# NVlabs/neuralrgbd

Measured on NVIDIA H100. Metric: depth frames/sec at 640x480x64-plane x4-view, higher is better.
Workload: dtype f32 (split-fp16 pair products: 22-bit significands, fp32 accumulate)

## Files before the change

neuralrgbd_b200/csrc/conv_f16.cu:

```cuda
#include <cuda.h>
#include <cuda_fp16.h>

#include "common.cuh"
#include "conv_wgmma.cuh"
#include "wgmma.cuh"
#include "../../include/nrgbd_dev.h"

namespace {

constexpr int WG_THREADS = 288;
constexpr int BKC = 32;

struct WgParams {
  float* y; const float* bias; double* stats;
  __half *y_hi, *y_lo;
  const float *aff_scale, *aff_shift, *res;
  const __half *res_hi, *res_lo;
  int relu;
  int N, Dz, Hy, Wx, tiles_x, tiles_y, n_tiles, wide;
  int cin_chunks, n_kz, n_tap, halo, in_stride, org_y, org_x;
  int Cout, c_first;
  int Dout, Hout, Wout, Cs_out, c_off, out_stride, out_off_y, out_off_x, leaky;
  int stages_a, stages_b, box_w, box_h;
  uint32_t a_tile_bytes, a_stage_bytes, a_tx_bytes, b_stage_bytes, wg_row16;
  uint32_t a_desc_hi, b_desc_hi;
  signed char dz[3];
  signed char dy[WG_MAX_TAP2D], dx[WG_MAX_TAP2D];
  unsigned short a_off16[WG_MAX_TAP2D];
  unsigned char wsel[3 * WG_MAX_TAP2D];
};

__device__ __forceinline__ uint32_t smem_u32(const void* p) { return (uint32_t)__cvta_generic_to_shared(p); }

__device__ __forceinline__ void mbar_init(uint32_t bar, uint32_t count) {
  asm volatile("mbarrier.init.shared::cta.b64 [%0], %1;" ::"r"(bar), "r"(count));
}
__device__ __forceinline__ void mbar_expect_tx(uint32_t bar, uint32_t bytes) {
  asm volatile("mbarrier.arrive.expect_tx.shared::cta.b64 _, [%0], %1;" ::"r"(bar), "r"(bytes) : "memory");
}
__device__ __forceinline__ void mbar_arrive(uint32_t bar) {
  asm volatile("mbarrier.arrive.shared::cta.b64 _, [%0];" ::"r"(bar) : "memory");
}
__device__ __forceinline__ void mbar_wait(uint32_t bar, uint32_t parity) {
  uint32_t done = 0;
#pragma unroll 1
  for (uint32_t it = 0; it < (1u << 27); ++it) {
    asm volatile(
        "{\n\t.reg .pred p;\n\t"
        "mbarrier.try_wait.parity.shared::cta.b64 p, [%1], %2;\n\t"
        "selp.b32 %0, 1, 0, p;\n\t}"
        : "=r"(done) : "r"(bar), "r"(parity) : "memory");
    if (done) return;
  }
  __trap();
}
__device__ __forceinline__ void tma_load_5d(uint32_t dst, const CUtensorMap* tm, uint32_t bar, int c0, int c1, int c2, int c3, int c4) {
  asm volatile(
      "cp.async.bulk.tensor.5d.shared::cluster.global.mbarrier::complete_tx::bytes [%0], [%1, {%3, %4, %5, %6, %7}], [%2];"
      ::"r"(dst), "l"((uint64_t)tm), "r"(bar), "r"(c0), "r"(c1), "r"(c2), "r"(c3), "r"(c4) : "memory");
}
__device__ __forceinline__ void tma_load_3d(uint32_t dst, const CUtensorMap* tm, uint32_t bar, int c0, int c1, int c2) {
  asm volatile(
      "cp.async.bulk.tensor.3d.shared::cluster.global.mbarrier::complete_tx::bytes [%0], [%1, {%3, %4, %5}], [%2];"
      ::"r"(dst), "l"((uint64_t)tm), "r"(bar), "r"(c0), "r"(c1), "r"(c2) : "memory");
}
__device__ __forceinline__ uint64_t wg_desc(uint32_t saddr, uint32_t hi) {
  return ((uint64_t)hi << 32) | (uint64_t)(((saddr & 0x3FFFFu) >> 4) | (1u << 16));
}

template <int BN, bool TF32>
__device__ __forceinline__ void wg_mma(float* d, uint64_t a, uint64_t b) {
  if constexpr (TF32) Wgmma<BN>::tf32(d, a, b); else Wgmma<BN>::f16(d, a, b);
}

template <int BN, bool TF32, int G, bool AFF>
__global__ void __launch_bounds__(WG_THREADS, BN <= 64 ? 2 : 1)
conv_wg_kernel(const __grid_constant__ CUtensorMap tm_a_hi, const __grid_constant__ CUtensorMap tm_a_lo,
               const __grid_constant__ CUtensorMap tm_b_hi, const __grid_constant__ CUtensorMap tm_b_lo, const WgParams p) {
  constexpr int RB = TF32 ? 128 : 64;
  constexpr int KS = TF32 ? 4 : 2;
  constexpr float SCALE = TF32 ? 1.f : 1.f / 2048.f;
  constexpr uint32_t B_HALF = (uint32_t)(G * BN * RB);
  constexpr int NJ = BN / 8;
  extern __shared__ __align__(1024) uint8_t smem_raw[];
  const uint32_t base = smem_u32(smem_raw);
  if (base & 1023u) __trap();
  const uint32_t b_ring = base + (uint32_t)p.stages_a * p.a_stage_bytes;
  const uint32_t sums_off = (uint32_t)p.stages_a * p.a_stage_bytes + (uint32_t)p.stages_b * p.b_stage_bytes;
  float* part = reinterpret_cast<float*>(smem_raw + sums_off);
  double* cta_sums = reinterpret_cast<double*>(smem_raw + sums_off + 8u * 2u * BN * 4u);
  const uint32_t bars = base + sums_off + 8u * 2u * BN * 4u + 2u * BN * 8u;
  const uint32_t bar_afull = bars, bar_aempty = bars + 64, bar_bfull = bars + 128, bar_bempty = bars + 192;
  const int warp = threadIdx.x >> 5, lane = threadIdx.x & 31;

  if (threadIdx.x == 0) {
    for (int s = 0; s < p.stages_a; ++s) { mbar_init(bar_afull + 8 * s, 1); mbar_init(bar_aempty + 8 * s, 8); }
    for (int s = 0; s < p.stages_b; ++s) { mbar_init(bar_bfull + 8 * s, 1); mbar_init(bar_bempty + 8 * s, 8); }
    asm volatile("fence.mbarrier_init.release.cluster;" ::: "memory");
  }
  if (threadIdx.x < 2 * BN) cta_sums[threadIdx.x] = 0.0;
  if constexpr (AFF) {
    const int c0 = p.c_first + (int)blockIdx.y * BN, t = threadIdx.x % BN;
    if (threadIdx.x < 2 * BN) part[threadIdx.x] = c0 + t < p.Cout ? __ldg((threadIdx.x < BN ? p.aff_scale : p.aff_shift) + c0 + t) : 0.f;
  }
  __syncthreads();

  const int th = p.wide ? 8 : 16, tw = p.wide ? 16 : 8;
  const int cbase = p.c_first + (int)blockIdx.y * BN;
  const int n_steps = p.n_kz * p.cin_chunks * (p.n_tap / G);

  if (warp == 8) {
    if (lane == 0) {
      int sa = 0, sb = 0;
      uint32_t pha = 0, phb = 0;
      for (int tile = blockIdx.x; tile < p.n_tiles; tile += gridDim.x) {
        int t = tile;
        const int ox0 = (t % p.tiles_x) * tw; t /= p.tiles_x;
        const int oy0 = (t % p.tiles_y) * th; t /= p.tiles_y;
        const int z0 = t % p.Dz, n0 = t / p.Dz;
        for (int kz = 0; kz < p.n_kz; ++kz) {
          const int cz = z0 + p.dz[kz];
          for (int cc = 0; cc < p.cin_chunks; ++cc) {
            for (int tap = 0; tap < p.n_tap; tap += G) {
              if (!p.halo || tap == 0) {
                const int cx = ox0 * p.in_stride + (p.halo ? p.org_x : (int)p.dx[tap]);
                const int cy = oy0 * p.in_stride + (p.halo ? p.org_y : (int)p.dy[tap]);
                mbar_wait(bar_aempty + 8 * sa, pha ^ 1u);
                mbar_expect_tx(bar_afull + 8 * sa, p.a_tx_bytes);
                const uint32_t dst = base + (uint32_t)sa * p.a_stage_bytes;
                tma_load_5d(dst, &tm_a_hi, bar_afull + 8 * sa, cc * BKC, cx, cy, cz, n0);
                tma_load_5d(dst + p.a_tile_bytes, &tm_a_lo, bar_afull + 8 * sa, cc * BKC, cx, cy, cz, n0);
                if (++sa == p.stages_a) { sa = 0; pha ^= 1u; }
              }
              mbar_wait(bar_bempty + 8 * sb, phb ^ 1u);
              mbar_expect_tx(bar_bfull + 8 * sb, 2 * B_HALF);
              const uint32_t dst = b_ring + (uint32_t)sb * p.b_stage_bytes;
              const int ws = p.wsel[kz * p.n_tap + tap];
              tma_load_3d(dst, &tm_b_hi, bar_bfull + 8 * sb, cc * BKC, cbase, ws);
              tma_load_3d(dst + B_HALF, &tm_b_lo, bar_bfull + 8 * sb, cc * BKC, cbase, ws);
              if (++sb == p.stages_b) { sb = 0; phb ^= 1u; }
            }
          }
        }
      }
    }
    return;
  }

  const int cw = warp >> 2, w4 = warp & 3;
  float acc_m[BN / 2], acc_c[BN / 2];
  const uint32_t wg_off = (uint32_t)cw * p.wg_row16 * 16u;
  int sa = 0, sb = 0, sa_cur = 0, tap = 0;
  uint32_t pha = 0, phb = 0;
  for (int tile = blockIdx.x; tile < p.n_tiles; tile += gridDim.x) {
#pragma unroll
    for (int k = 0; k < BN / 2; ++k) { acc_m[k] = 0.f; acc_c[k] = 0.f; }
    int rel_a = -1, rel_b = -1;
    for (int step = 0; step < n_steps; ++step) {
      const bool new_a = !p.halo || tap == 0;
      if (new_a) {
        mbar_wait(bar_afull + 8 * sa, pha);
        sa_cur = sa;
        if (++sa == p.stages_a) { sa = 0; pha ^= 1u; }
      }
      mbar_wait(bar_bfull + 8 * sb, phb);
      const uint32_t a_hi = base + (uint32_t)sa_cur * p.a_stage_bytes + wg_off;
      const uint32_t b_hi = b_ring + (uint32_t)sb * p.b_stage_bytes;
      asm volatile("wgmma.fence.sync.aligned;" ::: "memory");
#pragma unroll
      for (int g = 0; g < G; ++g) {
        const uint32_t ao = a_hi + (p.halo ? (uint32_t)p.a_off16[tap + g] * 16u : 0u);
#pragma unroll
        for (int ks = 0; ks < KS; ++ks) {
          const uint32_t ah = ao + 32u * ks, al = ah + p.a_tile_bytes;
          const uint32_t bh = b_hi + (uint32_t)(g * BN * RB) + 32u * ks, bl = bh + B_HALF;
          wg_mma<BN, TF32>(acc_m, wg_desc(ah, p.a_desc_hi), wg_desc(bh, p.b_desc_hi));
          wg_mma<BN, TF32>(acc_c, wg_desc(ah, p.a_desc_hi), wg_desc(bl, p.b_desc_hi));
          wg_mma<BN, TF32>(acc_c, wg_desc(al, p.a_desc_hi), wg_desc(bh, p.b_desc_hi));
        }
      }
      asm volatile("wgmma.commit_group.sync.aligned;" ::: "memory");
      asm volatile("wgmma.wait_group.sync.aligned 1;" ::: "memory");
      if (lane == 0) {
        if (rel_b >= 0) mbar_arrive(bar_bempty + 8 * rel_b);
        if (rel_a >= 0) mbar_arrive(bar_aempty + 8 * rel_a);
      }
      tap += G;
      const bool last_of_a = !p.halo || tap == p.n_tap;
      if (tap == p.n_tap) tap = 0;
      rel_b = sb; rel_a = last_of_a ? sa_cur : -1;
      if (++sb == p.stages_b) { sb = 0; phb ^= 1u; }
    }
    asm volatile("wgmma.wait_group.sync.aligned 0;" ::: "memory");
    if (lane == 0) {
      mbar_arrive(bar_bempty + 8 * rel_b);
      mbar_arrive(bar_aempty + 8 * rel_a);
    }

    int t = tile;
    const int ox0 = (t % p.tiles_x) * tw; t /= p.tiles_x;
    const int oy0 = (t % p.tiles_y) * th; t /= p.tiles_y;
    const int z0 = t % p.Dz, n0 = t / p.Dz;
    const int n_here = min(BN, p.Cout - cbase);
    const bool pair = p.y_hi != nullptr;
    const bool vec2 = ((p.Cs_out | (p.c_off + cbase)) & 1) == 0;
    float* dst_row[2] = {nullptr, nullptr};
    long long pix[2] = {0, 0};
    bool valid[2];
#pragma unroll
    for (int i = 0; i < 2; ++i) {
      const int r = 16 * w4 + (lane >> 2) + 8 * i;
      const int iy = oy0 + (r >> 3) + (p.wide ? 0 : 8 * cw), ix = ox0 + (r & 7) + (p.wide ? 8 * cw : 0);
      valid[i] = iy < p.Hy && ix < p.Wx;
      const int oy = iy * p.out_stride + p.out_off_y, ox = ix * p.out_stride + p.out_off_x;
      pix[i] = (((long long)n0 * p.Dout + z0) * p.Hout + oy) * p.Wout + ox;
      if (!pair) dst_row[i] = p.y + pix[i] * (long long)p.Cs_out + p.c_off + cbase;
    }
    if constexpr (AFF) {
#pragma unroll
      for (int k = 0; k < BN / 2; ++k) acc_m[k] = fmaf(acc_c[k], SCALE, acc_m[k]);
    }
    constexpr int NJ_PAIR = ((BN + 31) / 32) * 4;
    const int nj_store = pair ? NJ_PAIR : NJ;
#pragma unroll
    for (int j = 0; j < NJ_PAIR; ++j) {
      if (j >= nj_store) break;
      const int c = 8 * j + 2 * (lane & 3);
      float v[2][2];
#pragma unroll
      for (int i = 0; i < 2; ++i)
#pragma unroll
        for (int e = 0; e < 2; ++e) {
          float f = 0.f;
          if (j < NJ && c + e < n_here && valid[i]) {
            if constexpr (AFF) {
              f = fmaf(acc_m[4 * j + 2 * i + e], part[c + e], part[BN + c + e]);
            } else {
              f = fmaf(acc_c[4 * j + 2 * i + e], SCALE, acc_m[4 * j + 2 * i + e]);
              if (p.bias) f += __ldg(p.bias + cbase + c + e);
              if (p.leaky) f = f >= 0.f ? f : f * 0.01f;
            }
          }
          v[i][e] = f;
        }
#pragma unroll
      for (int i = 0; i < 2; ++i) {
        if (!valid[i]) continue;
        if constexpr (AFF) {
          const long long o = pix[i] * (long long)p.Cs_out + p.c_off + cbase + c;
#pragma unroll
          for (int e = 0; e < 2; ++e) {
            if (j < NJ && c + e < n_here) {
              if (p.res) v[i][e] += __ldg(p.res + o + e);
              else if (p.res_hi) v[i][e] += fmaf(__half2float(p.res_lo[o + e]), 1.f / 2048.f, __half2float(p.res_hi[o + e]));
              if (p.relu) v[i][e] = fmaxf(v[i][e], 0.f);
            }
          }
        }
        if (pair) {
          __half h0, l0, h1, l1;
          nrgbd_split_pair(v[i][0], h0, l0); nrgbd_split_pair(v[i][1], h1, l1);
          const long long o = pix[i] * (long long)p.Cs_out + cbase + c;
          *reinterpret_cast<__half2*>(p.y_hi + o) = __halves2half2(h0, h1);
          *reinterpret_cast<__half2*>(p.y_lo + o) = __halves2half2(l0, l1);
        } else if (vec2 && c + 1 < n_here) {
          *reinterpret_cast<float2*>(dst_row[i] + c) = make_float2(v[i][0], v[i][1]);
        } else {
          if (c < n_here) dst_row[i][c] = v[i][0];
          if (c + 1 < n_here) dst_row[i][c + 1] = v[i][1];
        }
      }
      if (!AFF && p.stats && j < NJ) {
        float s1[2], s2[2];
#pragma unroll
        for (int e = 0; e < 2; ++e) {
          s1[e] = v[0][e] + v[1][e];
          s2[e] = fmaf(v[0][e], v[0][e], v[1][e] * v[1][e]);
#pragma unroll
          for (int m = 4; m < 32; m <<= 1) {
            s1[e] += __shfl_xor_sync(0xffffffffu, s1[e], m);
            s2[e] += __shfl_xor_sync(0xffffffffu, s2[e], m);
          }
        }
        if (lane < 4) {
#pragma unroll
          for (int e = 0; e < 2; ++e) { part[(warp * 2) * BN + c + e] = s1[e]; part[(warp * 2 + 1) * BN + c + e] = s2[e]; }
        }
      }
    }
    if (!AFF && p.stats) {
      asm volatile("bar.sync 1, 256;" ::: "memory");
      const int c = threadIdx.x;
      if (c < n_here) {
        double a1 = 0.0, a2 = 0.0;
#pragma unroll
        for (int w = 0; w < 8; ++w) { a1 += (double)part[(w * 2) * BN + c]; a2 += (double)part[(w * 2 + 1) * BN + c]; }
        cta_sums[c] += a1; cta_sums[BN + c] += a2;
      }
      asm volatile("bar.sync 1, 256;" ::: "memory");
    }
  }
  const int c = threadIdx.x;
  if (!AFF && p.stats && c < min(BN, p.Cout - cbase) && (int)blockIdx.x < p.n_tiles) {
    atomicAdd(p.stats + cbase + c, cta_sums[c]);
    atomicAdd(p.stats + p.Cout + cbase + c, cta_sums[BN + c]);
  }
}

int g_h2_smem_cap_kb = 0;
int g_h2_flags = 0;

typedef CUresult (*EncodeTiledFn)(CUtensorMap*, CUtensorMapDataType, cuuint32_t, void*, const cuuint64_t*, const cuuint64_t*,
                                  const cuuint32_t*, const cuuint32_t*, CUtensorMapInterleave, CUtensorMapSwizzle,
                                  CUtensorMapL2promotion, CUtensorMapFloatOOBfill);
EncodeTiledFn get_encode() {
  static EncodeTiledFn fn = nullptr;
  if (!fn) {
    void* p = nullptr;
    cudaDriverEntryPointQueryResult q;
    if (cudaGetDriverEntryPoint("cuTensorMapEncodeTiled", &p, cudaEnableDefault, &q) == cudaSuccess && q == cudaDriverEntryPointSuccess)
      fn = (EncodeTiledFn)p;
  }
  return fn;
}

struct MapKey { const void* p; long long a; int b, c, d, e, f, g, h, i; };
struct MapEnt { MapKey k; CUtensorMap m; };
inline bool same_key(const MapKey& x, const MapKey& y) {
  return x.p == y.p && x.a == y.a && x.b == y.b && x.c == y.c && x.d == y.d && x.e == y.e && x.f == y.f && x.g == y.g && x.h == y.h && x.i == y.i;
}
thread_local MapEnt g_maps[1024];
inline unsigned key_slot(const MapKey& k) {
  unsigned long long h = (unsigned long long)k.p * 0x9E3779B97F4A7C15ull;
  h ^= (unsigned long long)(k.a * 73856093ll) ^ (unsigned long long)(k.b * 19349663u) ^ (unsigned long long)(k.c * 83492791u) ^
       (unsigned long long)(k.d * 2654435761u) ^ (unsigned long long)(k.e * 40503u) ^ (unsigned long long)(k.f * 2246822519u) ^
       (unsigned long long)(k.g * 3266489917u) ^ (unsigned long long)(k.h * 668265263u) ^ (unsigned long long)(k.i * 374761393u);
  return (unsigned)(h >> 40) & 1023u;
}

int encode_act_map(CUtensorMap* tm, const void* x, int esize, int N, int D, int H, int W, int C, int Cs, int box_w, int box_h, int stride) {
  MapKey k{x, (long long)N * 8 + esize, D, H, W, C, Cs, box_w, box_h, stride};
  MapEnt& e = g_maps[key_slot(k)];
  if (same_key(e.k, k) && e.k.p) { *tm = e.m; return NRGBD_OK; }
  EncodeTiledFn enc = get_encode();
  if (!enc) { nrgbd_set_error("cuTensorMapEncodeTiled unavailable"); return NRGBD_ERR_CUDA; }
  cuuint64_t dims[5] = {(cuuint64_t)C, (cuuint64_t)W, (cuuint64_t)H, (cuuint64_t)D, (cuuint64_t)N};
  cuuint64_t strides[4] = {(cuuint64_t)Cs * esize, (cuuint64_t)W * Cs * esize, (cuuint64_t)H * W * Cs * esize, (cuuint64_t)D * H * W * Cs * esize};
  cuuint32_t box[5] = {(cuuint32_t)BKC, (cuuint32_t)(box_w * stride), (cuuint32_t)(box_h * stride), 1, 1};
  cuuint32_t estr[5] = {1, (cuuint32_t)stride, (cuuint32_t)stride, 1, 1};
  CUresult r = enc(tm, esize == 2 ? CU_TENSOR_MAP_DATA_TYPE_FLOAT16 : CU_TENSOR_MAP_DATA_TYPE_FLOAT32, 5, const_cast<void*>(x), dims, strides, box,
                   estr, CU_TENSOR_MAP_INTERLEAVE_NONE, esize == 2 ? CU_TENSOR_MAP_SWIZZLE_64B : CU_TENSOR_MAP_SWIZZLE_128B,
                   CU_TENSOR_MAP_L2_PROMOTION_L2_256B, CU_TENSOR_MAP_FLOAT_OOB_FILL_NONE);
  if (r != CUDA_SUCCESS) { nrgbd_set_error("cuTensorMapEncodeTiled(activation, esize %d) failed: %d", esize, (int)r); return NRGBD_ERR_CUDA; }
  e.k = k; e.m = *tm;
  return NRGBD_OK;
}

int encode_w_map(CUtensorMap* tm, const void* w, int esize, long long tap_stride, int taps, int Cout_pad, int Cin_pad, int BN, int G) {
  MapKey k{w, tap_stride * 8 + esize, taps, Cout_pad, Cin_pad, BN, G, -7, -7, -7};
  MapEnt& e = g_maps[key_slot(k)];
  if (same_key(e.k, k) && e.k.p) { *tm = e.m; return NRGBD_OK; }
  EncodeTiledFn enc = get_encode();
  if (!enc) { nrgbd_set_error("cuTensorMapEncodeTiled unavailable"); return NRGBD_ERR_CUDA; }
  cuuint64_t dims[3] = {(cuuint64_t)Cin_pad, (cuuint64_t)Cout_pad, (cuuint64_t)taps};
  cuuint64_t strides[2] = {(cuuint64_t)Cin_pad * esize, (cuuint64_t)tap_stride * esize};
  cuuint32_t box[3] = {(cuuint32_t)BKC, (cuuint32_t)BN, (cuuint32_t)G};
  cuuint32_t estr[3] = {1, 1, 1};
  CUresult r = enc(tm, esize == 2 ? CU_TENSOR_MAP_DATA_TYPE_FLOAT16 : CU_TENSOR_MAP_DATA_TYPE_FLOAT32, 3, const_cast<void*>(w), dims, strides, box,
                   estr, CU_TENSOR_MAP_INTERLEAVE_NONE, esize == 2 ? CU_TENSOR_MAP_SWIZZLE_64B : CU_TENSOR_MAP_SWIZZLE_128B,
                   CU_TENSOR_MAP_L2_PROMOTION_L2_256B, CU_TENSOR_MAP_FLOAT_OOB_FILL_NONE);
  if (r != CUDA_SUCCESS) { nrgbd_set_error("cuTensorMapEncodeTiled(weights, esize %d) failed: %d", esize, (int)r); return NRGBD_ERR_CUDA; }
  e.k = k; e.m = *tm;
  return NRGBD_OK;
}

inline uint32_t round_up(uint32_t v, uint32_t m) { return (v + m - 1) / m * m; }

typedef void (*WgKernel)(const CUtensorMap, const CUtensorMap, const CUtensorMap, const CUtensorMap, const WgParams);

template <bool TF32, int G, bool AFF = false>
WgKernel pick_kernel(int BN) {
  switch (BN) {
    case 16: return conv_wg_kernel<16, TF32, G, AFF>;
    case 32: return conv_wg_kernel<32, TF32, G, AFF>;
    case 48: return conv_wg_kernel<48, TF32, G, AFF>;
    case 64: return conv_wg_kernel<64, TF32, G, AFF>;
    case 80: return conv_wg_kernel<80, TF32, G, AFF>;
    case 96: return conv_wg_kernel<96, TF32, G, AFF>;
    case 112: return conv_wg_kernel<112, TF32, G, AFF>;
    case 128: return conv_wg_kernel<128, TF32, G, AFF>;
  }
  return nullptr;
}

int launch_chunks(const WgConv& c, WgParams p, int BN, int n_chunks, int c_first, cudaStream_t st) {
  const bool tf32 = c.tf32 != 0;
  const int esize = tf32 ? 4 : 2, RB = BKC * esize;
  p.c_first = c_first;
  int G = 1;
  if (p.halo && p.n_tap % 3 == 0 && !(g_h2_flags & 128)) {
    bool consecutive = true;
    for (int t = 1; t < p.n_kz * p.n_tap; ++t) consecutive = consecutive && c.wsel[t] == c.wsel[t - 1] + 1;
    if (consecutive) G = 3;
  }
  const size_t extra = (size_t)8 * 2 * BN * 4 + (size_t)2 * BN * 8 + 256;
  auto plan = [&](size_t cap, int g, int& sa, int& sb) {
    const size_t b_stage = (size_t)2 * g * BN * RB;
    sa = 2;
    if (cap < extra + 2 * (size_t)p.a_stage_bytes + 2 * b_stage) return false;
    sb = (int)((cap - extra - 2 * (size_t)p.a_stage_bytes) / b_stage);
    if (sb > 8) sb = 8;
    if (sb >= 6 && cap >= extra + 3 * (size_t)p.a_stage_bytes + 4 * b_stage) { sa = 3; sb = (int)((cap - extra - 3 * (size_t)p.a_stage_bytes) / b_stage); if (sb > 8) sb = 8; }
    return true;
  };
  size_t cap = g_h2_smem_cap_kb > 0 ? (size_t)g_h2_smem_cap_kb * 1024 : (BN <= 64 ? 115712 - 1024 : 232448);
  int sa = 0, sb = 0;
  bool ok = plan(cap, G, sa, sb);
  if (!ok && G == 3) { G = 1; ok = plan(cap, G, sa, sb); }
  if (!ok) { cap = 232448; ok = plan(cap, G, sa, sb); }
  if (!ok) { nrgbd_set_error("conv_wgmma: tile does not fit the shared-memory pipeline"); return NRGBD_ERR_UNSUPPORTED; }
  p.stages_a = sa; p.stages_b = sb;
  p.b_stage_bytes = (uint32_t)(2 * G * BN * RB);
  const size_t smem = (size_t)sa * p.a_stage_bytes + (size_t)sb * p.b_stage_bytes + extra;
  CUtensorMap tb_hi, tb_lo;
  int rc = encode_w_map(&tb_hi, c.w_hi, esize, c.w_tap_stride, c.n_wslices, c.Cout_pad, c.Cin_pad, BN, G);
  if (rc == NRGBD_OK) rc = encode_w_map(&tb_lo, c.w_lo, esize, c.w_tap_stride, c.n_wslices, c.Cout_pad, c.Cin_pad, BN, G);
  if (rc != NRGBD_OK) return rc;
  CUtensorMap ta_hi, ta_lo;
  rc = encode_act_map(&ta_hi, c.x_hi, esize, c.N, c.Din, c.Hin, c.Win, c.Cin_pad, c.Cs_in, p.box_w, p.box_h, p.in_stride);
  if (rc == NRGBD_OK) rc = encode_act_map(&ta_lo, c.x_lo, esize, c.N, c.Din, c.Hin, c.Win, c.Cin_pad, c.Cs_in, p.box_w, p.box_h, p.in_stride);
  if (rc != NRGBD_OK) return rc;
  const bool aff = p.aff_scale != nullptr;
  if (aff && tf32) { nrgbd_set_error("conv_wgmma: the affine epilogue is built for split-fp16 operands only"); return NRGBD_ERR_UNSUPPORTED; }
  WgKernel fn = aff ? (G == 3 ? pick_kernel<false, 3, true>(BN) : pick_kernel<false, 1, true>(BN))
                    : tf32 ? (G == 3 ? pick_kernel<true, 3>(BN) : pick_kernel<true, 1>(BN))
                           : (G == 3 ? pick_kernel<false, 3>(BN) : pick_kernel<false, 1>(BN));
  if (!fn) { nrgbd_set_error("conv_wgmma: unsupported chunk width %d", BN); return NRGBD_ERR_UNSUPPORTED; }
  static size_t configured[2][2][2][8] = {};
  size_t& conf = configured[aff][tf32][G == 3][BN / 16 - 1];
  if (smem > conf) {
    cudaError_t e = cudaFuncSetAttribute(fn, cudaFuncAttributeMaxDynamicSharedMemorySize, (int)smem);
    if (e != cudaSuccess) { nrgbd_set_error("conv_wgmma: cannot opt in to %zu bytes of shared memory: %s", smem, cudaGetErrorString(e)); return NRGBD_ERR_CUDA; }
    conf = smem;
  }
  int grid_x = p.n_tiles;
  if (!(g_h2_flags & 32)) {
    const int per_sm = (int)std::min<size_t>(BN <= 64 ? 2 : 1, 233472 / (smem + 1024));
    grid_x = std::min(grid_x, ceil_div(nrgbd_sm_count() * per_sm, n_chunks));
  }
  fn<<<dim3((unsigned)grid_x, (unsigned)n_chunks), WG_THREADS, smem, st>>>(ta_hi, ta_lo, tb_hi, tb_lo, p);
  return NRGBD_OK;
}

}

int conv_wgmma(const WgConv& c, cudaStream_t st) {
  NRGBD_REQUIRE(c.n_tap >= 1 && c.n_tap <= WG_MAX_TAP2D && c.n_kz >= 1 && c.n_kz <= 3 && c.Cin_pad % BKC == 0 && c.Cout_pad % 16 == 0,
                "unsupported convolution shape");
  const int esize = c.tf32 ? 4 : 2, RB = BKC * esize;
  WgParams p{};
  p.y = c.y; p.bias = c.bias; p.stats = c.stats;
  p.y_hi = reinterpret_cast<__half*>(c.y_hi); p.y_lo = reinterpret_cast<__half*>(c.y_lo);
  p.aff_scale = c.aff_scale; p.aff_shift = c.aff_shift; p.res = c.res; p.relu = c.relu;
  p.res_hi = reinterpret_cast<const __half*>(c.res_hi); p.res_lo = reinterpret_cast<const __half*>(c.res_lo);
  p.N = c.N; p.Dz = c.Din; p.Hy = c.Hy; p.Wx = c.Wx;
  const long long pad_tall = (long long)ceil_div(c.Hy, 16) * ceil_div(c.Wx, 8), pad_wide = (long long)ceil_div(c.Hy, 8) * ceil_div(c.Wx, 16);
  p.wide = (pad_wide < pad_tall && !(g_h2_flags & 8)) ? 1 : 0;
  const int TH = p.wide ? 8 : 16, TW = p.wide ? 16 : 8;
  p.tiles_x = ceil_div(c.Wx, TW); p.tiles_y = ceil_div(c.Hy, TH);
  NRGBD_REQUIRE((long long)p.N * p.Dz * p.tiles_x * p.tiles_y < (1ll << 31), "too many output tiles");
  p.n_tiles = p.N * p.Dz * p.tiles_x * p.tiles_y;
  p.cin_chunks = c.Cin_pad / BKC; p.n_kz = c.n_kz; p.n_tap = c.n_tap; p.in_stride = c.in_stride;
  p.Cout = c.Cout; p.Dout = c.Dout; p.Hout = c.Hout; p.Wout = c.Wout; p.Cs_out = c.Cs_out; p.c_off = c.c_off;
  p.out_stride = c.out_stride; p.out_off_y = c.out_off_y; p.out_off_x = c.out_off_x; p.leaky = c.leaky;
  for (int a = 0; a < 3; ++a) p.dz[a] = c.dz[a];
  for (int t = 0; t < WG_MAX_TAP2D; ++t) { p.dy[t] = c.dy[t]; p.dx[t] = c.dx[t]; }
  for (int t = 0; t < 3 * WG_MAX_TAP2D; ++t) p.wsel[t] = c.wsel[t];
  p.halo = (c.in_stride == 1 && c.n_tap > 1 && !(g_h2_flags & 4)) ? 1 : 0;
  int pitch = TW, halo_rows = TH;
  if (p.halo) {
    int min_dy = 127, max_dy = -127, min_dx = 127, max_dx = -127;
    for (int t = 0; t < c.n_tap; ++t) {
      min_dy = c.dy[t] < min_dy ? c.dy[t] : min_dy; max_dy = c.dy[t] > max_dy ? c.dy[t] : max_dy;
      min_dx = c.dx[t] < min_dx ? c.dx[t] : min_dx; max_dx = c.dx[t] > max_dx ? c.dx[t] : max_dx;
    }
    pitch = TW + (max_dx - min_dx); halo_rows = TH + (max_dy - min_dy);
    if (pitch > TW + 16 || halo_rows > TH + 16) { p.halo = 0; pitch = TW; halo_rows = TH; }
    else {
      p.org_y = min_dy; p.org_x = min_dx;
      for (int t = 0; t < c.n_tap; ++t) p.a_off16[t] = (unsigned short)((((c.dy[t] - min_dy) * pitch + (c.dx[t] - min_dx)) * RB) >> 4);
    }
  }
  const uint32_t swz_mode = c.tf32 ? 1u : 2u;
  p.a_desc_hi = (uint32_t)((pitch * RB) >> 4) | (swz_mode << 30);
  p.b_desc_hi = (uint32_t)((8 * RB) >> 4) | (swz_mode << 30);
  p.wg_row16 = (uint32_t)((8 * (p.wide ? 1 : pitch) * RB) >> 4);
  p.box_w = pitch; p.box_h = halo_rows;
  p.a_tx_bytes = 2u * (uint32_t)(halo_rows * pitch * RB);
  p.a_tile_bytes = round_up((uint32_t)(halo_rows * pitch * RB), 1024);
  p.a_stage_bytes = 2 * p.a_tile_bytes;
  const int n_chunks = (c.Cout_pad + 127) / 128;
  const int BN = c.Cout_pad < 128 ? c.Cout_pad : 128;
  const int BN_last = c.Cout_pad - (n_chunks - 1) * BN;
  const int n_full = BN_last == BN ? n_chunks : n_chunks - 1;
  int rc = launch_chunks(c, p, BN, n_full, 0, st);
  if (rc == NRGBD_OK && n_full < n_chunks) rc = launch_chunks(c, p, BN_last, 1, n_full * BN, st);
  return rc;
}

namespace {
__device__ __forceinline__ void split_pair(float a, __half& hi, __half& lo) { nrgbd_split_pair(a, hi, lo); }

__global__ void __launch_bounds__(256)
split_f16_pair_kernel(const float4* __restrict__ x, long long n4, uint2* __restrict__ hi, uint2* __restrict__ lo) {
  for (long long i = (long long)blockIdx.x * blockDim.x + threadIdx.x; i < n4; i += (long long)gridDim.x * blockDim.x) {
    const float4 v = x[i];
    __half h[4], l[4];
    split_pair(v.x, h[0], l[0]); split_pair(v.y, h[1], l[1]); split_pair(v.z, h[2], l[2]); split_pair(v.w, h[3], l[3]);
    uint2 ho, lo2;
    ho.x = (uint32_t)__half_as_ushort(h[0]) | ((uint32_t)__half_as_ushort(h[1]) << 16);
    ho.y = (uint32_t)__half_as_ushort(h[2]) | ((uint32_t)__half_as_ushort(h[3]) << 16);
    lo2.x = (uint32_t)__half_as_ushort(l[0]) | ((uint32_t)__half_as_ushort(l[1]) << 16);
    lo2.y = (uint32_t)__half_as_ushort(l[2]) | ((uint32_t)__half_as_ushort(l[3]) << 16);
    hi[i] = ho; lo[i] = lo2;
  }
}

__global__ void pack_weight_h2_kernel(const float* __restrict__ w, int kind, int Cout, int Cin, int taps, int Cin_pad, int Cout_pad,
                                      __half* __restrict__ out) {
  long long i = (long long)blockIdx.x * blockDim.x + threadIdx.x;
  long long n = (long long)taps * Cin_pad * Cout_pad;
  if (i >= n) return;
  int ci = (int)(i % Cin_pad);
  int co = (int)((i / Cin_pad) % Cout_pad);
  int t = (int)(i / ((long long)Cout_pad * Cin_pad));
  float v = 0.f;
  if (co < Cout && ci < Cin) v = kind == 0 ? w[((long long)co * Cin + ci) * taps + t] : w[((long long)ci * Cout + co) * taps + t];
  __half h, l;
  split_pair(v, h, l);
  const long long tile = (long long)Cout_pad * Cin_pad;
  out[(long long)t * 2 * tile + (long long)co * Cin_pad + ci] = h;
  out[(long long)t * 2 * tile + tile + (long long)co * Cin_pad + ci] = l;
}

}

extern "C" {

void nrgbd_dev_conv_h2_set_flags(int flags) { g_h2_flags = flags; }
void nrgbd_dev_conv_h2_set_smem_cap_kb(int kb) { g_h2_smem_cap_kb = kb; }

int nrgbd_conv_h2_plan(int Cin, int Cout, int* Cin_pad, int* Cout_pad, int* BN) {
  if (Cin < 1 || Cout < 1) return 0;
  const int c16 = (Cout + 15) / 16 * 16;
  if (Cin_pad) *Cin_pad = (Cin + 31) / 32 * 32;
  if (Cout_pad) *Cout_pad = c16;
  if (BN) *BN = c16 < 128 ? c16 : 128;
  return 1;
}

int nrgbd_split_f16_pair(const float* x, long long n, void* hi, void* lo, cudaStream_t st) {
  NRGBD_REQUIRE(x && hi && lo && n > 0 && n % 4 == 0, "bad arguments");
  long long blocks = (n / 4 + 255) / 256;
  if (blocks > nrgbd_sm_count() * 16ll) blocks = nrgbd_sm_count() * 16ll;
  split_f16_pair_kernel<<<(unsigned)blocks, 256, 0, st>>>(reinterpret_cast<const float4*>(x), n / 4, reinterpret_cast<uint2*>(hi),
                                                         reinterpret_cast<uint2*>(lo));
  NRGBD_COUNT(1);
  NRGBD_LAUNCH_CHECK();
  return NRGBD_OK;
}

int nrgbd_pack_conv_weight_h2(const float* w, int transposed, int Cout, int Cin, int taps, int Cin_pad, int Cout_pad, void* out,
                              cudaStream_t st) {
  NRGBD_REQUIRE(w && out && Cout > 0 && Cin > 0 && taps > 0 && Cin_pad >= Cin && Cout_pad >= Cout, "bad arguments");
  long long n = (long long)taps * Cin_pad * Cout_pad;
  pack_weight_h2_kernel<<<ceil_div(n, 256), 256, 0, st>>>(w, transposed ? 1 : 0, Cout, Cin, taps, Cin_pad, Cout_pad, reinterpret_cast<__half*>(out));
  NRGBD_COUNT(1);
  NRGBD_LAUNCH_CHECK();
  return NRGBD_OK;
}

static int conv_nhwc_h2_impl(const void* x_hi, const void* x_lo, int N, int Din, int Hin, int Win, int Cin_pad, int Cs_in, const void* w,
                             const float* bias, int Cout, int Cout_pad, int BN, int kd, int kh, int kw, int stride, int pad, int dilation, float* y,
                             void* y_hi, void* y_lo, int Hout, int Wout, int Cs_out, int c_off, int leaky, double* stats, cudaStream_t st,
                             const WgConv* aff = nullptr);

int nrgbd_conv_nhwc_h2(const void* x_hi, const void* x_lo, int N, int Din, int Hin, int Win, int Cin_pad, int Cs_in, const void* w,
                       const float* bias, int Cout, int Cout_pad, int BN, int kd, int kh, int kw, int stride, int pad, int dilation, float* y,
                       int Hout, int Wout, int Cs_out, int c_off, int leaky, double* stats, cudaStream_t st) {
  NRGBD_REQUIRE(y, "null pointer");
  return conv_nhwc_h2_impl(x_hi, x_lo, N, Din, Hin, Win, Cin_pad, Cs_in, w, bias, Cout, Cout_pad, BN, kd, kh, kw, stride, pad, dilation, y, nullptr,
                           nullptr, Hout, Wout, Cs_out, c_off, leaky, stats, st);
}

int nrgbd_conv_nhwc_h2_pair(const void* x_hi, const void* x_lo, int N, int Din, int Hin, int Win, int Cin_pad, int Cs_in, const void* w,
                            const float* bias, int Cout, int Cout_pad, int BN, int kd, int kh, int kw, int stride, int pad, int dilation,
                            void* y_hi, void* y_lo, int Hout, int Wout, int Cs_out, int leaky, cudaStream_t st) {
  NRGBD_REQUIRE(y_hi && y_lo, "null pointer");
  return conv_nhwc_h2_impl(x_hi, x_lo, N, Din, Hin, Win, Cin_pad, Cs_in, w, bias, Cout, Cout_pad, BN, kd, kh, kw, stride, pad, dilation, nullptr, y_hi,
                           y_lo, Hout, Wout, Cs_out, 0, leaky, nullptr, st);
}

static int conv_nhwc_h2_impl(const void* x_hi, const void* x_lo, int N, int Din, int Hin, int Win, int Cin_pad, int Cs_in, const void* w,
                             const float* bias, int Cout, int Cout_pad, int BN, int kd, int kh, int kw, int stride, int pad, int dilation, float* y,
                             void* y_hi, void* y_lo, int Hout, int Wout, int Cs_out, int c_off, int leaky, double* stats, cudaStream_t st,
                             const WgConv* aff) {
  NRGBD_REQUIRE(x_hi && x_lo && w, "null pointer");
  NRGBD_REQUIRE(Cin_pad % 32 == 0 && Cin_pad >= 32 && Cin_pad <= Cs_in && Cs_in % 8 == 0 && Cout_pad % 16 == 0 && Cout <= Cout_pad && Cout > Cout_pad - 16 &&
                    BN == (Cout_pad < 128 ? Cout_pad : 128), "channel counts not supported by the f16-pair tensor-core path");
  NRGBD_REQUIRE(kd >= 1 && kd <= 3 && kh * kw <= WG_MAX_TAP2D && stride >= 1 && stride <= 8, "unsupported filter");
  NRGBD_REQUIRE(Hout == (Hin + 2 * pad - dilation * (kh - 1) - 1) / stride + 1 &&
                    Wout == (Win + 2 * pad - dilation * (kw - 1) - 1) / stride + 1, "output extent mismatch");
  if (y_hi) {
    NRGBD_REQUIRE(Cs_out % 32 == 0 && Cs_out >= Cout_pad && c_off == 0 && stats == nullptr && (((uintptr_t)y_hi | (uintptr_t)y_lo) & 15) == 0 && y_lo,
                  "pair output needs Cs_out % 32 == 0, c_off == 0 and no statistics");
  }
  WgConv c{};
  c.tf32 = 0;
  c.x_hi = x_hi; c.x_lo = x_lo; c.N = N; c.Din = Din; c.Hin = Hin; c.Win = Win; c.Cin_pad = Cin_pad; c.Cs_in = Cs_in;
  c.w_hi = w; c.w_lo = reinterpret_cast<const __half*>(w) + (long long)Cout_pad * Cin_pad; c.w_tap_stride = 2ll * Cout_pad * Cin_pad;
  c.n_wslices = kd * kh * kw; c.Cout_pad = Cout_pad;
  c.bias = bias; c.stats = stats; c.y = y; c.y_hi = y_hi; c.y_lo = y_lo;
  c.Cout = Cout; c.Dout = Din; c.Hout = Hout; c.Wout = Wout; c.Cs_out = Cs_out; c.c_off = c_off;
  c.out_stride = 1; c.out_off_y = 0; c.out_off_x = 0; c.leaky = leaky;
  if (aff) { c.aff_scale = aff->aff_scale; c.aff_shift = aff->aff_shift; c.res = aff->res; c.res_hi = aff->res_hi; c.res_lo = aff->res_lo; c.relu = aff->relu; }
  c.Hy = Hout; c.Wx = Wout; c.in_stride = stride; c.n_kz = kd; c.n_tap = kh * kw;
  for (int a = 0; a < kd; ++a) c.dz[a] = (signed char)(a - kd / 2);
  int t = 0;
  for (int b = 0; b < kh; ++b)
    for (int e = 0; e < kw; ++e) { c.dy[t] = (signed char)(b * dilation - pad); c.dx[t] = (signed char)(e * dilation - pad); ++t; }
  for (int a = 0; a < kd * kh * kw; ++a) c.wsel[a] = (unsigned char)a;
  int rc = conv_wgmma(c, st);
  if (rc != NRGBD_OK) return rc;
  NRGBD_COUNT(1);
  NRGBD_LAUNCH_CHECK();
  return NRGBD_OK;
}

int nrgbd_conv_nhwc_h2_affine(const void* x_hi, const void* x_lo, int N, int Din, int Hin, int Win, int Cin_pad, int Cs_in, const void* w,
                              int Cout, int Cout_pad, int BN, int kd, int kh, int kw, int stride, int pad, int dilation,
                              const float* scale, const float* shift, const float* res, const void* res_hi, const void* res_lo, int relu,
                              float* y, void* y_hi, void* y_lo, int Hout, int Wout, int Cs_out, int c_off, cudaStream_t st) {
  NRGBD_REQUIRE(scale && shift, "null scale / shift");
  NRGBD_REQUIRE((y != nullptr) != (y_hi != nullptr) && (y_hi == nullptr) == (y_lo == nullptr), "the output is either fp32 (y) or a pair (y_hi, y_lo)");
  NRGBD_REQUIRE((res_hi == nullptr) == (res_lo == nullptr) && !(res && res_hi), "the residual is either an fp32 tensor or an operand pair");
  WgConv aff{};
  aff.aff_scale = scale; aff.aff_shift = shift; aff.res = res; aff.res_hi = res_hi; aff.res_lo = res_lo; aff.relu = relu ? 1 : 0;
  return conv_nhwc_h2_impl(x_hi, x_lo, N, Din, Hin, Win, Cin_pad, Cs_in, w, nullptr, Cout, Cout_pad, BN, kd, kh, kw, stride, pad, dilation, y,
                           y_hi, y_lo, Hout, Wout, Cs_out, c_off, 0, nullptr, st, &aff);
}

int nrgbd_conv_transpose2d_k4s2_nhwc_h2(const void* x_hi, const void* x_lo, int N, int Hin, int Win, int Cin_pad, int Cs_in, const void* w,
                                        const float* bias, int Cout, int Cout_pad, int BN, float* y, int Cs_out, int c_off, int leaky,
                                        cudaStream_t st) {
  NRGBD_REQUIRE(x_hi && x_lo && w && y, "null pointer");
  NRGBD_REQUIRE(Cin_pad % 32 == 0 && Cin_pad >= 32 && Cin_pad <= Cs_in && Cs_in % 8 == 0 && Cout_pad % 16 == 0 && Cout <= Cout_pad && Cout > Cout_pad - 16 &&
                    BN == (Cout_pad < 128 ? Cout_pad : 128), "channel counts not supported by the f16-pair tensor-core path");
  const int kys[2][2] = {{1, 3}, {0, 2}};
  const int dys[2][2] = {{0, -1}, {1, 0}};
  for (int py = 0; py < 2; ++py)
    for (int px = 0; px < 2; ++px) {
      WgConv c{};
      c.tf32 = 0;
      c.x_hi = x_hi; c.x_lo = x_lo; c.N = N; c.Din = 1; c.Hin = Hin; c.Win = Win; c.Cin_pad = Cin_pad; c.Cs_in = Cs_in;
      c.w_hi = w; c.w_lo = reinterpret_cast<const __half*>(w) + (long long)Cout_pad * Cin_pad; c.w_tap_stride = 2ll * Cout_pad * Cin_pad;
      c.n_wslices = 16; c.Cout_pad = Cout_pad;
      c.bias = bias; c.stats = nullptr; c.y = y;
      c.Cout = Cout; c.Dout = 1; c.Hout = 2 * Hin; c.Wout = 2 * Win; c.Cs_out = Cs_out; c.c_off = c_off;
      c.out_stride = 2; c.out_off_y = py; c.out_off_x = px; c.leaky = leaky;
      c.Hy = Hin; c.Wx = Win; c.in_stride = 1; c.n_kz = 1; c.n_tap = 4;
      int t = 0;
      for (int a = 0; a < 2; ++a)
        for (int b = 0; b < 2; ++b) {
          c.dy[t] = (signed char)dys[py][a]; c.dx[t] = (signed char)dys[px][b];
          c.wsel[t] = (unsigned char)(kys[py][a] * 4 + kys[px][b]); ++t;
        }
      int rc = conv_wgmma(c, st);
      if (rc != NRGBD_OK) return rc;
    }
  NRGBD_COUNT(4);
  NRGBD_LAUNCH_CHECK();
  return NRGBD_OK;
}

}
```

Before: 100.6.

## Add specialized 64-output-channel persistent conv kernel with resident weights

Adds a dedicated kernel for stride-1 halo convolutions with 64 output channels, fp16 split pairs, and taps grouped in rows of three. It uses one producer warpgroup and two consumer warpgroups that alternate tiles, so one tile's epilogue overlaps the other's MMAs. When the weights fit, they are loaded once into shared memory and kept resident across tiles. The goal is to cut repeated weight TMA traffic and epilogue stalls for these layers, at the cost of a large new code path and a forced tall tile shape.

Measured after the change: 103.3, median of 6. +2.7%, better.

```diff
diff --git a/neuralrgbd_b200/csrc/conv_f16.cu b/neuralrgbd_b200/csrc/conv_f16.cu
--- a/neuralrgbd_b200/csrc/conv_f16.cu
+++ b/neuralrgbd_b200/csrc/conv_f16.cu
@@ -22,6 +22,7 @@
   int Cout, c_first;
   int Dout, Hout, Wout, Cs_out, c_off, out_stride, out_off_y, out_off_x, leaky;
   int stages_a, stages_b, box_w, box_h;
+  int w_resident;
   uint32_t a_tile_bytes, a_stage_bytes, a_tx_bytes, b_stage_bytes, wg_row16;
   uint32_t a_desc_hi, b_desc_hi;
   signed char dz[3];
@@ -304,6 +305,230 @@
   if (!AFF && p.stats && c < min(BN, p.Cout - cbase) && (int)blockIdx.x < p.n_tiles) {
     atomicAdd(p.stats + cbase + c, cta_sums[c]);
     atomicAdd(p.stats + p.Cout + cbase + c, cta_sums[BN + c]);
+  }
+}
+
+constexpr int C64_THREADS = 384;
+
+template <int TH, int OUT, bool FULL>
+__device__ __forceinline__ void c64_epilogue(const WgParams& p, const float* acc_m, const float* acc_c, const float* bias, int ch, int lane,
+                                             int n_here, int ox0, int oy0, long long plane, double* bn) {
+  static_assert(OUT != 2 || TH % 2 == 0, "BatchNorm blocks are row pairs");
+  constexpr float SCALE = 1.f / 2048.f;
+  const int cbase = p.c_first;
+  const int ix0 = ox0 + 2 * (lane & 3);
+  const int odd = (lane >> 2) & 1;
+  const bool has_bias = p.bias != nullptr, leaky = p.leaky != 0;
+  float top[2][2];
+#pragma unroll
+  for (int j = 0; j < TH; ++j) {
+    const int iy = oy0 + j;
+    const long long row = (plane * p.Hout + iy) * p.Wout;
+#pragma unroll
+    for (int i = 0; i < 2; ++i) {
+      const int c = ch + 8 * i;
+      float v[2];
+#pragma unroll
+      for (int e = 0; e < 2; ++e) {
+        float f = fmaf(acc_c[4 * j + 2 * i + e], SCALE, acc_m[4 * j + 2 * i + e]);
+        if (has_bias) f += bias[i];
+        if (leaky) f = f >= 0.f ? f : f * 0.01f;
+        v[e] = (FULL || (c < n_here && iy < p.Hy && ix0 + e < p.Wx)) ? f : 0.f;
+      }
+      if (OUT == 2) {
+        if ((j & 1) == 0) {
+          top[i][0] = v[0]; top[i][1] = v[1];
+        } else {
+          float s1 = (top[i][0] + v[0]) + (top[i][1] + v[1]);
+          float s2 = fmaf(top[i][0], top[i][0], v[0] * v[0]) + fmaf(top[i][1], top[i][1], v[1] * v[1]);
+#pragma unroll
+          for (int m = 1; m < 4; m <<= 1) {
+            s1 += __shfl_xor_sync(0xffffffffu, s1, m);
+            s2 += __shfl_xor_sync(0xffffffffu, s2, m);
+          }
+          if ((lane & 3) == 0) { bn[c] += (double)s1; bn[64 + c] += (double)s2; }
+        }
+      }
+      const float r = __shfl_xor_sync(0xffffffffu, odd ? v[0] : v[1], 4);
+      const float lo_c = odd ? r : v[0], hi_c = odd ? v[1] : r;
+      const int c0 = c & ~1, ix = ix0 + odd;
+      if (!FULL && (iy >= p.Hy || ix >= p.Wx)) continue;
+      const long long pix = row + ix;
+      if (OUT == 1) {
+        __half h0, l0, h1, l1;
+        nrgbd_split_pair(lo_c, h0, l0); nrgbd_split_pair(hi_c, h1, l1);
+        const long long o = pix * (long long)p.Cs_out + cbase + c0;
+        *reinterpret_cast<__half2*>(p.y_hi + o) = __halves2half2(h0, h1);
+        *reinterpret_cast<__half2*>(p.y_lo + o) = __halves2half2(l0, l1);
+      } else {
+        float* dst = p.y + pix * (long long)p.Cs_out + p.c_off + cbase + c0;
+        if (FULL || ((((p.Cs_out | (p.c_off + cbase)) & 1) == 0) && c0 + 1 < n_here)) {
+          *reinterpret_cast<float2*>(dst) = make_float2(lo_c, hi_c);
+        } else {
+          if (c0 < n_here) dst[0] = lo_c;
+          if (c0 + 1 < n_here) dst[1] = hi_c;
+        }
+      }
+    }
+  }
+}
+
+__global__ void __launch_bounds__(C64_THREADS, 1)
+conv_c64_kernel(const __grid_constant__ CUtensorMap tm_a_hi, const __grid_constant__ CUtensorMap tm_a_lo,
+                const __grid_constant__ CUtensorMap tm_b_hi, const __grid_constant__ CUtensorMap tm_b_lo, const WgParams p) {
+  constexpr int RB = 64, KS = 2, BN = 64, TH = 16, N = 8 * TH, G = 3;
+  constexpr uint32_t B_HALF = (uint32_t)(G * BN * RB);
+  extern __shared__ __align__(1024) uint8_t smem_raw[];
+  const uint32_t base = smem_u32(smem_raw);
+  if (base & 1023u) __trap();
+  const uint32_t b_ring = base + (uint32_t)p.stages_a * p.a_stage_bytes;
+  const uint32_t sums_off = (uint32_t)p.stages_a * p.a_stage_bytes + (uint32_t)p.stages_b * p.b_stage_bytes;
+  double* bn_sums = reinterpret_cast<double*>(smem_raw + sums_off);
+  const uint32_t bars = base + sums_off + 4u * BN * 8u;
+  const uint32_t bar_afull = bars, bar_aempty = bars + 64, bar_bfull = bars + 128, bar_bempty = bars + 192;
+  const int lane = threadIdx.x & 31;
+
+  if (threadIdx.x == 0) {
+    for (int s = 0; s < p.stages_a; ++s) { mbar_init(bar_afull + 8 * s, 1); mbar_init(bar_aempty + 8 * s, 4); }
+    for (int s = 0; s < p.stages_b; ++s) { mbar_init(bar_bfull + 8 * s, 1); mbar_init(bar_bempty + 8 * s, 4); }
+    asm volatile("fence.mbarrier_init.release.cluster;" ::: "memory");
+  }
+  if (threadIdx.x < 4 * BN) bn_sums[threadIdx.x] = 0.0;
+  __syncthreads();
+
+  const int cbase = p.c_first;
+  const int n_a = p.n_kz * p.cin_chunks;
+  const int n_steps = n_a * (p.n_tap / G);
+
+  if (threadIdx.x < 128) {
+    asm volatile("setmaxnreg.dec.sync.aligned.u32 40;" ::: "memory");
+    if (threadIdx.x == 0) {
+      int sa = 0, sb = 0;
+      uint32_t pha = 0, phb = 0;
+      for (int tile = blockIdx.x; tile < p.n_tiles; tile += gridDim.x) {
+        int t = tile;
+        const int ox0 = (t % p.tiles_x) * 8; t /= p.tiles_x;
+        const int oy0 = (t % p.tiles_y) * TH; t /= p.tiles_y;
+        const int z0 = t % p.Dz, n0 = t / p.Dz;
+        for (int kz = 0; kz < p.n_kz; ++kz) {
+          const int cz = z0 + p.dz[kz];
+          for (int cc = 0; cc < p.cin_chunks; ++cc) {
+            mbar_wait(bar_aempty + 8 * sa, pha ^ 1u);
+            mbar_expect_tx(bar_afull + 8 * sa, p.a_tx_bytes);
+            const uint32_t dst = base + (uint32_t)sa * p.a_stage_bytes;
+            tma_load_5d(dst, &tm_a_hi, bar_afull + 8 * sa, cc * BKC, ox0 + p.org_x, oy0 + p.org_y, cz, n0);
+            tma_load_5d(dst + p.a_tile_bytes, &tm_a_lo, bar_afull + 8 * sa, cc * BKC, ox0 + p.org_x, oy0 + p.org_y, cz, n0);
+            if (++sa == p.stages_a) { sa = 0; pha ^= 1u; }
+            if (p.w_resident && tile != (int)blockIdx.x) continue;
+            for (int tap = 0; tap < p.n_tap; tap += G) {
+              mbar_wait(bar_bempty + 8 * sb, phb ^ 1u);
+              mbar_expect_tx(bar_bfull + 8 * sb, 2 * B_HALF);
+              const uint32_t wdst = b_ring + (uint32_t)sb * p.b_stage_bytes;
+              const int ws = p.wsel[kz * p.n_tap + tap];
+              tma_load_3d(wdst, &tm_b_hi, bar_bfull + 8 * sb, cc * BKC, cbase, ws);
+              tma_load_3d(wdst + B_HALF, &tm_b_lo, bar_bfull + 8 * sb, cc * BKC, cbase, ws);
+              if (++sb == p.stages_b) { sb = 0; phb ^= 1u; }
+            }
+          }
+        }
+      }
+    }
+    return;
+  }
+
+  asm volatile("setmaxnreg.inc.sync.aligned.u32 232;" ::: "memory");
+  const int cw = (threadIdx.x >> 7) - 1, w4 = (threadIdx.x >> 5) & 3;
+  const int n_here = min(BN, p.Cout - cbase);
+  const int ch = 16 * w4 + (lane >> 2);
+  float bias[2] = {0.f, 0.f};
+#pragma unroll
+  for (int i = 0; i < 2; ++i)
+    if (p.bias && ch + 8 * i < n_here) bias[i] = __ldg(p.bias + cbase + ch + 8 * i);
+  const int n_local = (int)blockIdx.x < p.n_tiles ? (p.n_tiles - (int)blockIdx.x + (int)gridDim.x - 1) / (int)gridDim.x : 0;
+  auto advance = [](int& s, uint32_t& ph, int n, int stages) {
+    s += n;
+    while (s >= stages) { s -= stages; ph ^= 1u; }
+  };
+  int sa = 0, sb = 0;
+  uint32_t pha = 0, phb = 0;
+  advance(sa, pha, cw * n_a, p.stages_a);
+  advance(sb, phb, cw * n_steps, p.stages_b);
+  float acc_m[N / 2], acc_c[N / 2];
+  const bool pair = p.y_hi != nullptr;
+  const bool vec2 = ((p.Cs_out | (p.c_off + cbase)) & 1) == 0;
+  for (int k = cw; k < n_local; k += 2) {
+    const int tile = (int)blockIdx.x + k * (int)gridDim.x;
+#pragma unroll
+    for (int q = 0; q < N / 2; ++q) { acc_m[q] = 0.f; acc_c[q] = 0.f; }
+    if (k > 0) asm volatile("bar.sync %0, 256;" ::"r"(2 + cw) : "memory");
+    int rel_a = -1, rel_b = -1, sa_cur = 0, tap = 0;
+    for (int step = 0; step < n_steps; ++step) {
+      if (tap == 0) {
+        mbar_wait(bar_afull + 8 * sa, pha);
+        sa_cur = sa;
+        if (++sa == p.stages_a) { sa = 0; pha ^= 1u; }
+      }
+      const int slot_b = p.w_resident ? step : sb;
+      mbar_wait(bar_bfull + 8 * slot_b, p.w_resident ? 0u : phb);
+      const uint32_t a_hi = base + (uint32_t)sa_cur * p.a_stage_bytes;
+      const uint32_t b_hi = b_ring + (uint32_t)slot_b * p.b_stage_bytes;
+      asm volatile("wgmma.fence.sync.aligned;" ::: "memory");
+#pragma unroll
+      for (int g = 0; g < G; ++g) {
+        const uint32_t ao = a_hi + (uint32_t)p.a_off16[tap + g] * 16u;
+#pragma unroll
+        for (int ks = 0; ks < KS; ++ks) {
+          const uint32_t xh = ao + 32u * ks, xl = xh + p.a_tile_bytes;
+          const uint32_t wh = b_hi + (uint32_t)(g * BN * RB) + 32u * ks, wl = wh + B_HALF;
+          Wgmma<N>::f16(acc_m, wg_desc(wh, p.b_desc_hi), wg_desc(xh, p.a_desc_hi));
+          Wgmma<N>::f16(acc_c, wg_desc(wl, p.b_desc_hi), wg_desc(xh, p.a_desc_hi));
+          Wgmma<N>::f16(acc_c, wg_desc(wh, p.b_desc_hi), wg_desc(xl, p.a_desc_hi));
+        }
+      }
+      asm volatile("wgmma.commit_group.sync.aligned;" ::: "memory");
+      asm volatile("wgmma.wait_group.sync.aligned 1;" ::: "memory");
+      if (lane == 0) {
+        if (rel_b >= 0) mbar_arrive(bar_bempty + 8 * rel_b);
+        if (rel_a >= 0) mbar_arrive(bar_aempty + 8 * rel_a);
+      }
+      tap += G;
+      const bool last_of_a = tap == p.n_tap;
+      if (last_of_a) tap = 0;
+      rel_b = p.w_resident ? -1 : sb; rel_a = last_of_a ? sa_cur : -1;
+      if (++sb == p.stages_b) { sb = 0; phb ^= 1u; }
+    }
+    if (k + 1 < n_local) asm volatile("bar.arrive %0, 256;" ::"r"(2 + (cw ^ 1)) : "memory");
+    asm volatile("wgmma.wait_group.sync.aligned 0;" ::: "memory");
+    if (lane == 0) {
+      if (rel_b >= 0) mbar_arrive(bar_bempty + 8 * rel_b);
+      mbar_arrive(bar_aempty + 8 * rel_a);
+    }
+    advance(sa, pha, n_a, p.stages_a);
+    advance(sb, phb, n_steps, p.stages_b);
+
+    int t = tile;
+    const int ox0 = (t % p.tiles_x) * 8; t /= p.tiles_x;
+    const int oy0 = (t % p.tiles_y) * TH; t /= p.tiles_y;
+    const long long plane = (long long)(t / p.Dz) * p.Dout + t % p.Dz;
+    const bool full = n_here == BN && vec2 && oy0 + TH <= p.Hy && ox0 + 8 <= p.Wx;
+    if (pair) {
+      if (full) c64_epilogue<TH, 1, true>(p, acc_m, acc_c, bias, ch, lane, n_here, ox0, oy0, plane, bn_sums + cw * 2 * BN);
+      else c64_epilogue<TH, 1, false>(p, acc_m, acc_c, bias, ch, lane, n_here, ox0, oy0, plane, bn_sums + cw * 2 * BN);
+    } else if (p.stats) {
+      if (full) c64_epilogue<16, 2, true>(p, acc_m, acc_c, bias, ch, lane, n_here, ox0, oy0, plane, bn_sums + cw * 2 * BN);
+      else c64_epilogue<16, 2, false>(p, acc_m, acc_c, bias, ch, lane, n_here, ox0, oy0, plane, bn_sums + cw * 2 * BN);
+    } else {
+      if (full) c64_epilogue<TH, 0, true>(p, acc_m, acc_c, bias, ch, lane, n_here, ox0, oy0, plane, bn_sums + cw * 2 * BN);
+      else c64_epilogue<TH, 0, false>(p, acc_m, acc_c, bias, ch, lane, n_here, ox0, oy0, plane, bn_sums + cw * 2 * BN);
+    }
+  }
+  if (p.stats && (int)blockIdx.x < p.n_tiles) {
+    asm volatile("bar.sync 4, 256;" ::: "memory");
+    const int c = threadIdx.x - 128;
+    if (c < n_here) {
+      atomicAdd(p.stats + cbase + c, bn_sums[c] + bn_sums[2 * BN + c]);
+      atomicAdd(p.stats + p.Cout + cbase + c, bn_sums[BN + c] + bn_sums[3 * BN + c]);
+    }
   }
 }
 
@@ -452,6 +677,44 @@
   return NRGBD_OK;
 }
 
+int launch_c64(const WgConv& c, WgParams p, cudaStream_t st) {
+  constexpr int BN = 64, RB = 64;
+  constexpr int G = 3;
+  p.c_first = 0;
+  const size_t extra = (size_t)4 * BN * 8 + 256;
+  const size_t cap = g_h2_smem_cap_kb > 0 ? (size_t)g_h2_smem_cap_kb * 1024 : 232448;
+  const size_t b_stage = (size_t)2 * G * BN * RB;
+  int sa = 3, sb = 0;
+  const int n_steps = p.n_kz * p.cin_chunks * (p.n_tap / G);
+  p.w_resident = n_steps <= 8 && cap >= extra + 3 * (size_t)p.a_stage_bytes + (size_t)n_steps * b_stage ? 1 : 0;
+  if (p.w_resident) {
+    sb = n_steps;
+  } else {
+    if (cap < extra + 3 * (size_t)p.a_stage_bytes + 2 * b_stage) sa = 2;
+    if (cap < extra + (size_t)sa * p.a_stage_bytes + 2 * b_stage) { nrgbd_set_error("conv_wgmma: tile does not fit the shared-memory pipeline"); return NRGBD_ERR_UNSUPPORTED; }
+    sb = (int)std::min<size_t>(8, (cap - extra - (size_t)sa * p.a_stage_bytes) / b_stage);
+  }
+  p.stages_a = sa; p.stages_b = sb;
+  p.b_stage_bytes = (uint32_t)b_stage;
+  const size_t smem = (size_t)sa * p.a_stage_bytes + (size_t)sb * b_stage + extra;
+  CUtensorMap tb_hi, tb_lo, ta_hi, ta_lo;
+  int rc = encode_w_map(&tb_hi, c.w_hi, 2, c.w_tap_stride, c.n_wslices, c.Cout_pad, c.Cin_pad, BN, G);
+  if (rc == NRGBD_OK) rc = encode_w_map(&tb_lo, c.w_lo, 2, c.w_tap_stride, c.n_wslices, c.Cout_pad, c.Cin_pad, BN, G);
+  if (rc == NRGBD_OK) rc = encode_act_map(&ta_hi, c.x_hi, 2, c.N, c.Din, c.Hin, c.Win, c.Cin_pad, c.Cs_in, p.box_w, p.box_h, 1);
+  if (rc == NRGBD_OK) rc = encode_act_map(&ta_lo, c.x_lo, 2, c.N, c.Din, c.Hin, c.Win, c.Cin_pad, c.Cs_in, p.box_w, p.box_h, 1);
+  if (rc != NRGBD_OK) return rc;
+  WgKernel fn = conv_c64_kernel;
+  static size_t conf = 0;
+  if (smem > conf) {
+    cudaError_t e = cudaFuncSetAttribute(fn, cudaFuncAttributeMaxDynamicSharedMemorySize, (int)smem);
+    if (e != cudaSuccess) { nrgbd_set_error("conv_wgmma: cannot opt in to %zu bytes of shared memory: %s", smem, cudaGetErrorString(e)); return NRGBD_ERR_CUDA; }
+    conf = smem;
+  }
+  const int grid_x = (g_h2_flags & 32) ? p.n_tiles : std::min(p.n_tiles, nrgbd_sm_count());
+  fn<<<(unsigned)grid_x, C64_THREADS, smem, st>>>(ta_hi, ta_lo, tb_hi, tb_lo, p);
+  return NRGBD_OK;
+}
+
 }
 
 int conv_wgmma(const WgConv& c, cudaStream_t st) {
@@ -464,8 +727,18 @@
   p.aff_scale = c.aff_scale; p.aff_shift = c.aff_shift; p.res = c.res; p.relu = c.relu;
   p.res_hi = reinterpret_cast<const __half*>(c.res_hi); p.res_lo = reinterpret_cast<const __half*>(c.res_lo);
   p.N = c.N; p.Dz = c.Din; p.Hy = c.Hy; p.Wx = c.Wx;
+  int min_dy = 127, max_dy = -127, min_dx = 127, max_dx = -127;
+  for (int t = 0; t < c.n_tap; ++t) {
+    min_dy = c.dy[t] < min_dy ? c.dy[t] : min_dy; max_dy = c.dy[t] > max_dy ? c.dy[t] : max_dy;
+    min_dx = c.dx[t] < min_dx ? c.dx[t] : min_dx; max_dx = c.dx[t] > max_dx ? c.dx[t] : max_dx;
+  }
+  p.halo = (c.in_stride == 1 && c.n_tap > 1 && !(g_h2_flags & 4) && max_dx - min_dx <= 16 && max_dy - min_dy <= 16) ? 1 : 0;
+  bool rows3 = c.n_tap % 3 == 0 && !(g_h2_flags & 128);
+  for (int t = 1; t < c.n_tap; ++t) rows3 = rows3 && c.wsel[t] == c.wsel[t - 1] + 1;
+  const bool c64 = p.halo && rows3 && c.n_kz == 1 && !c.tf32 && !c.aff_scale && c.Cout_pad == 64 && c.out_stride == 1 &&
+                   !(g_h2_flags & 16);
   const long long pad_tall = (long long)ceil_div(c.Hy, 16) * ceil_div(c.Wx, 8), pad_wide = (long long)ceil_div(c.Hy, 8) * ceil_div(c.Wx, 16);
-  p.wide = (pad_wide < pad_tall && !(g_h2_flags & 8)) ? 1 : 0;
+  p.wide = (!c64 && pad_wide < pad_tall && !(g_h2_flags & 8)) ? 1 : 0;
   const int TH = p.wide ? 8 : 16, TW = p.wide ? 16 : 8;
   p.tiles_x = ceil_div(c.Wx, TW); p.tiles_y = ceil_div(c.Hy, TH);
   NRGBD_REQUIRE((long long)p.N * p.Dz * p.tiles_x * p.tiles_y < (1ll << 31), "too many output tiles");
@@ -476,20 +749,11 @@
   for (int a = 0; a < 3; ++a) p.dz[a] = c.dz[a];
   for (int t = 0; t < WG_MAX_TAP2D; ++t) { p.dy[t] = c.dy[t]; p.dx[t] = c.dx[t]; }
   for (int t = 0; t < 3 * WG_MAX_TAP2D; ++t) p.wsel[t] = c.wsel[t];
-  p.halo = (c.in_stride == 1 && c.n_tap > 1 && !(g_h2_flags & 4)) ? 1 : 0;
   int pitch = TW, halo_rows = TH;
   if (p.halo) {
-    int min_dy = 127, max_dy = -127, min_dx = 127, max_dx = -127;
-    for (int t = 0; t < c.n_tap; ++t) {
-      min_dy = c.dy[t] < min_dy ? c.dy[t] : min_dy; max_dy = c.dy[t] > max_dy ? c.dy[t] : max_dy;
-      min_dx = c.dx[t] < min_dx ? c.dx[t] : min_dx; max_dx = c.dx[t] > max_dx ? c.dx[t] : max_dx;
-    }
     pitch = TW + (max_dx - min_dx); halo_rows = TH + (max_dy - min_dy);
-    if (pitch > TW + 16 || halo_rows > TH + 16) { p.halo = 0; pitch = TW; halo_rows = TH; }
-    else {
-      p.org_y = min_dy; p.org_x = min_dx;
-      for (int t = 0; t < c.n_tap; ++t) p.a_off16[t] = (unsigned short)((((c.dy[t] - min_dy) * pitch + (c.dx[t] - min_dx)) * RB) >> 4);
-    }
+    p.org_y = min_dy; p.org_x = min_dx;
+    for (int t = 0; t < c.n_tap; ++t) p.a_off16[t] = (unsigned short)((((c.dy[t] - min_dy) * pitch + (c.dx[t] - min_dx)) * RB) >> 4);
   }
   const uint32_t swz_mode = c.tf32 ? 1u : 2u;
   p.a_desc_hi = (uint32_t)((pitch * RB) >> 4) | (swz_mode << 30);
@@ -499,6 +763,7 @@
   p.a_tx_bytes = 2u * (uint32_t)(halo_rows * pitch * RB);
   p.a_tile_bytes = round_up((uint32_t)(halo_rows * pitch * RB), 1024);
   p.a_stage_bytes = 2 * p.a_tile_bytes;
+  if (c64) return launch_c64(c, p, st);
   const int n_chunks = (c.Cout_pad + 127) / 128;
   const int BN = c.Cout_pad < 128 ? c.Cout_pad : 128;
   const int BN_last = c.Cout_pad - (n_chunks - 1) * BN;
```
